# aask1357/fastenhancer

Measured on AMD Instinct MI355X. Metric: audio frames/sec (hop=256, 16kHz) FastEnhancer_B, higher is better.
Workload: dtype f32

## Files before the change

### fastenhancer_amd/_lib.py

```python
from __future__ import annotations

import ctypes
import os
from ctypes import POINTER, byref, c_char_p, c_double, c_float, c_int, c_longlong, c_size_t, c_void_p

HERE = os.path.dirname(os.path.abspath(__file__))
LIB_PATH = os.environ.get("FASTENHANCER_HIP_LIB") or os.path.join(HERE, "libfastenhancer_hip.so")
FE_MAX_KERNELS = 8

FE_OK = 0
FE_ARCH_FASTENHANCER = 0
FE_ARCH_BSRNN = 1
FE_ARCH_FSPEN = 2
FE_ARCH_LISENNET = 3
FE_OFFLINE_AUTO, FE_OFFLINE_FRAME_WALK, FE_OFFLINE_TIME_BATCHED = 0, 1, 2
FE_STEP_KERNEL_WAVES4, FE_STEP_KERNEL_WG8, FE_STEP_KERNEL_WG8_PERSIST = 0, 1, 2
FE_ACT_SILU, FE_ACT_RELU, FE_ACT_LEAKY_RELU, FE_ACT_ELU, FE_ACT_GELU, FE_ACT_GELU_TANH = 0, 1, 2, 3, 4, 5
FE_MASK_NONE, FE_MASK_SIGMOID, FE_MASK_TANH = 0, 1, 2
FE_AUDIO_F32, FE_AUDIO_S16 = 0, 1


class fe_config(ctypes.Structure):
    _fields_ = [
        ("arch", c_int), ("n_fft", c_int), ("hop_size", c_int), ("win_size", c_int),
# ... 64 lines not shown
    "fe_offline": (c_int, [c_void_p, c_void_p, c_int, c_int, c_void_p, c_void_p, c_void_p, c_void_p]),
    "fe_offline_ragged_work_floats": (c_size_t, [c_void_p, c_int, c_int]),
    "fe_offline_ragged": (c_int, [c_void_p, c_void_p, c_size_t, POINTER(c_int), c_int, c_void_p, c_size_t, c_void_p, c_void_p, c_void_p]),
    "fe_stft_step": (c_int, [c_void_p, c_void_p, c_size_t, c_void_p, c_void_p, c_void_p, c_int, c_void_p]),
    "fe_istft_step": (c_int, [c_void_p, c_void_p, c_void_p, c_void_p, c_void_p, c_size_t, c_int, c_void_p]),
    "fe_stft_offline": (c_int, [c_void_p, c_void_p, c_int, c_int, c_int, c_int, c_void_p, c_void_p]),
    "fe_istft_offline": (c_int, [c_void_p, c_void_p, c_int, c_int, c_int, c_int, c_void_p, c_void_p, c_void_p]),
    "fe_flops_per_frame": (c_double, [c_void_p]),
    "fe_debug_stages": (c_int, [c_void_p]),
    "fe_debug_stage": (c_int, [c_void_p, c_int, POINTER(c_char_p), POINTER(c_int), POINTER(c_int), POINTER(c_size_t)]),
    "fe_debug_floats": (c_size_t, [c_void_p]),
    "fe_debug_step": (c_int, [c_void_p, c_void_p, c_size_t, c_void_p, c_void_p, c_size_t, c_int, c_void_p, c_void_p]),
    "fe_profile_step": (c_int, [c_void_p, c_void_p, c_size_t, c_void_p, c_void_p, c_size_t, c_int, c_int, c_void_p, c_void_p]),
    "fe_debug_poison_lds": (c_int, [c_void_p]),
    "fe_debug_pack_weights": (c_int, [c_void_p, c_void_p, c_size_t, c_void_p, c_size_t, POINTER(c_size_t)]),
    "fe_last_error": (c_char_p, []),
    "fe_version": (c_char_p, []),
    "fe_build_key": (c_char_p, []),
}

_lib = None


class FEError(RuntimeError):
    pass


def load() -> ctypes.CDLL:
    global _lib
    if _lib is not None:
# ... 24 lines not shown
```

### fastenhancer_amd/csrc/fe_api.hip

```cpp
#include <hip/hip_runtime.h>

#include <algorithm>
#include <cmath>
#include <cstdarg>
#include <cstdio>
#include <cstdlib>
#include <cstring>
#include <string>
#include <vector>

#include "../../include/fastenhancer_hip.h"
#include "fe_fragments.h"
#include "fe_impl.h"
#include "bsrnn_kernels.hip.h"
#include "fspen_kernels.hip.h"
#include "lisennet_kernels.hip.h"
#include "stft_kernels.hip.h"

namespace fe {
namespace {
struct KernelLog { const char* name[16]; int n; };
thread_local KernelLog g_klog{};
}
void note_kernel(const char* name) {
// ... 408 lines not shown
            for (int g = 0; g < 3; ++g) {
                pack_1x1(o.blk_wih[k] + g * gsz, wih + (size_t)g * C2 * C2, C2, C2);
                pack_1x1(o.blk_whh[k] + g * gsz, whh + (size_t)g * C2 * C2, C2, C2);
                p.raw(o.blk_bih[k] + g * bsz, C2, bih + g * C2);
                p.raw(o.blk_bhh[k] + g * bsz, C2, bhh + g * C2);
            }
        }
        if (o.u8_gx[k] != 0) {
            const float* wih = S(key("rnn.weight_ih_l0"));
            const float* whh = S(key("rnn.weight_hh_l0"));
            const float* bih = S(key("rnn.bias_ih_l0"));
            const float* bhh = S(key("rnn.bias_hh_l0"));
            const int NG = C2 / 16, R = C2 % 16, NT = 3 * NG + 1, KS = C2 / 4;
            auto pack_u8 = [&](int off, int ntiles, const float* w, auto&& wrow, auto&& bias, auto&& rscale) {
                p.tiles(off, ntiles, KS, [&](int t, int c, int kk) { const int row = wrow(t, c); return row >= 0 ? w[(size_t)row * C2 + kk] * rscale(row) : 0.0f; });
                p.rows((size_t)off + (size_t)ntiles * KS * 64, ntiles, [&](int t, int c) { const int row = wrow(t, c); return row >= 0 ? bias(t, c) * rscale(row) : 0.0f; });
            };
            auto one = [](int) { return 1.0f; };
            auto gscale = [&](int row) { return row < 2 * C2 ? fe::kGateRZ : fe::kGateN; };
            auto grow = [&](int t, int c) -> int {
                if (t < 3 * NG) return (t % 3) * C2 + 16 * (t / 3) + c;
                return c < 3 * R ? (c / R) * C2 + 16 * NG + c % R : -1;
            };
            auto shared = [&](int t) { return t < 3 * NG && t % 3 < 2; };
            pack_u8(o.u8_gx[k], NT, wih, grow, [&](int t, int c) { const int r = grow(t, c); return bih[r] + (shared(t) ? bhh[r] : 0.0f); }, gscale);
            pack_u8(o.u8_gh[k], NT, whh, grow, [&](int t, int c) { const int r = grow(t, c); return shared(t) ? 0.0f : bhh[r]; }, gscale);
            auto plain = [&](int ncols) { return [ncols](int t, int c) { return 16 * t + c < ncols ? 16 * t + c : -1; }; };
            const float* f1b = S(key("rnn_fc.bias"));
            const float* f2b = S(key("attn_fc.bias"));
            pack_u8(o.u8_f1[k], fe::ceil_div(C2, 16), S(key("rnn_fc.weight")), plain(C2), [&](int t, int c) { return f1b[16 * t + c]; }, one);
            pack_1x1(o.u8_q[k], S(key("attn.qkv.weight")), C2, 3 * C2);
// ... 486 lines not shown
    return rc;
}

int fe_debug_pack_weights(fe_handle* h, const float* blob_host, size_t nfloats, float* out_host, size_t capacity, size_t* packed_floats) {
    if (!h || !blob_host) return fail(FE_ERR_INVALID_ARG, "null argument");
    if (nfloats != h->blob_floats) return fail(FE_ERR_INVALID_ARG, "blob has %zu floats, expected %zu", nfloats, h->blob_floats);
    std::vector<float> packed;
    const int rc = pack_blob(h, blob_host, &packed);
    if (rc != FE_OK) return rc;
    if (out_host && capacity < packed.size()) return fail(FE_ERR_INVALID_ARG, "output holds %zu floats, the packed buffer has %zu", capacity, packed.size());
    if (packed_floats) *packed_floats = packed.size();
    if (out_host) std::memcpy(out_host, packed.data(), packed.size() * sizeof(float));
    return FE_OK;
}

static const char* banks_unsupported(const fe_handle* h) {
    switch (h->cfg.arch) {
    case FE_ARCH_BSRNN: return "BSRNN";
    case FE_ARCH_FSPEN: return "FSPEN";
    case FE_ARCH_LISENNET: return "LiSenNet";
    default: return h->d.BD ? "noncausal FastEnhancer" : nullptr;
    }
}

int fe_weight_banks(const fe_handle* h) { return h ? h->n_banks : 0; }

int fe_set_weight_banks(fe_handle* h, int n_banks, void* stream) {
    if (!h) return fail(FE_ERR_INVALID_ARG, "null handle");
    if (n_banks < 1 || n_banks > FE_MAX_WEIGHT_BANKS)
        return fail(FE_ERR_INVALID_ARG, "fe_set_weight_banks: n_banks %d outside [1, FE_MAX_WEIGHT_BANKS = %d]", n_banks, FE_MAX_WEIGHT_BANKS);
// ... 1311 lines not shown
```

### fastenhancer_amd/csrc/fe_fragments.h

```cpp
#pragma once

#include <cstddef>
#include <vector>

namespace fe {
namespace frag {

enum Order { kPlain, kK4 };

constexpr size_t plain_index(int tile, int KS, int ks, int lane) { return ((size_t)tile * KS + ks) * 64 + lane; }
constexpr size_t k4_index(int tile, int KS, int ks, int lane) { return (((size_t)tile * (KS / 4) + ks / 4) * 64 + lane) * 4 + ks % 4; }
constexpr int lane_r(int lane) { return lane % 16; }
constexpr int lane_k(int ks, int lane) { return 4 * ks + lane / 16; }

struct Buffer {
    std::vector<float> v;
    explicit Buffer(size_t floats = 0) : v(floats, 0.0f) {}
    float& operator[](size_t i) { return v[i]; }
    size_t size() const { return v.size(); }
    int alloc(size_t n) {
        const size_t off = (v.size() + 63) & ~(size_t)63;
        v.resize(off + n, 0.0f);
        return (int)off;
    }
// ... 12 lines not shown
                    v[off + (O == kK4 ? k4_index(t, KS, ks, lane) : plain_index(t, KS, ks, lane))] = f(t, lane_r(lane), lane_k(ks, lane));
    }
    template <Order O = kPlain, class F>
    void pack_a(size_t off, int Mrows, int K, F&& Amk) {
        tiles<O>(off, (Mrows + 15) / 16, K / 4, [&](int t, int r, int k) { return 16 * t + r < Mrows ? Amk(16 * t + r, k) : 0.0f; });
    }
    template <Order O = kPlain, class F>
    void pack_b(size_t off, int K, int Ncols, F&& Bkn) {
        tiles<O>(off, (Ncols + 15) / 16, K / 4, [&](int t, int r, int k) { return 16 * t + r < Ncols ? Bkn(k, 16 * t + r) : 0.0f; });
    }
    template <class F>
    void rows(size_t off, int NT, F&& f) {
        for (int t = 0; t < NT; ++t)
            for (int r = 0; r < 16; ++r) v[off + (size_t)t * 16 + r] = f(t, r);
    }
    template <class TileMap>
    void regroup_k4(size_t dst, size_t src, int ntiles, int KS, int k0, int nk, TileMap&& src_tile) {
        for (int t = 0; t < ntiles; ++t)
            for (int ks = 0; ks < nk; ++ks)
                for (int lane = 0; lane < 64; ++lane)
                    v[dst + (size_t)t * nk * 64 + (ks < nk / 4 * 4 ? k4_index(0, nk, ks, lane) : plain_index(0, nk, ks, lane))] =
                        v[src + plain_index(src_tile(t), KS, k0 + ks, lane)];
    }
    void regroup_k4(size_t dst, size_t src, int ntiles, int KS, int k0, int nk) { regroup_k4(dst, src, ntiles, KS, k0, nk, [](int t) { return t; }); }
};

}
}
```

### fastenhancer_amd/csrc/fe_frame8.hip.h

```cpp
#pragma once
#include "fe_kernels.hip.h"

namespace fe {

constexpr int kThreads8 = 512;
constexpr int kWaves8 = 8;

template <class S>
struct Wg8 {
    using L = Lds<S>;
    static constexpr bool MDFT = (S::NFFT == 512) || (S::C1 < 128);
    static constexpr bool OK0 = L::STAGED && L::SKIPS_LDS && S::GFLAT && S::KT == 1 && S::LOW == 0 && !S::FRNN && !S::TATT && !S::LN && !S::BIDIR &&
                               S::G8P && S::MTC == 4 && S::MT2 == 2 && MDFT && !L::PERHEAD && S::NFFT == kThreads8 && S::NTPW2 == 1;
    static constexpr int NTA = (S::NTC + 1) / 2, NTB = S::NTC - NTA;
    static constexpr int N2A = (S::NT2 + 1) / 2, N2B = S::NT2 - N2A;
    static constexpr int NPW = ceil_div(ceil_div(Pack<S>::umax(), 256), kWaves8);
    static constexpr int HPT = ceil_div(S::F2 * S::C2, kThreads8);
    static constexpr int SLOT = S::U8_SLOT;
    static constexpr int WB0 = L::NOSTAGE_TOTAL, WB1 = WB0 + 2 * SLOT;
    static constexpr int LDM = 13;
    static constexpr int MXB = L::NOSTAGE_TOTAL + 4 * SLOT, MX_FLOATS = round_up(4 * 16 * LDM + 8, 4), MXF = MXB + 4 * 16 * LDM;
    static constexpr int HST = MXB + MX_FLOATS;
    static constexpr bool HSTASH = (size_t)(HST + S::KB * S::F2 * S::C2) * 4 <= 160 * 1024;
    static constexpr size_t BYTES = (size_t)(HST + (HSTASH ? S::KB * S::F2 * S::C2 : 0)) * 4;
// ... 11 lines not shown
    return q;
}
__device__ __forceinline__ f32x4 lds_v4(const LdsF* p) { return *reinterpret_cast<const LdsV4*>(p); }
template <int NPW, int NP>
struct Stage8 : StageSide<NPW, NP, kWaves8> {
    LdsF* w;
    __device__ __forceinline__ void commit() const {
        using B = StageSide<NPW, NP, kWaves8>;
#pragma unroll
        for (int i = 0; i < B::NPI; ++i) {
            const int p = this->j->wave + kWaves8 * i;
            if (kWaves8 * i + kWaves8 - 1 < NP || p < NP) *reinterpret_cast<LdsV4*>(w + i * (kWaves8 * 256)) = this->j->r[i];
        }
    }
};
__device__ __forceinline__ f32x4 lds_splat(const float* p) {
    const float b = *p;
    return f32x4{b, b, b, b};
}

template <class S, int NT, int J0, int KS, int NCOLS, int LDO, bool ACT, class AF, class BF, class BI, class SIDE>
__device__ __forceinline__ void conv8(AF&& af, BF&& bf, BI&& bias, const SIDE& side, LdsF* dst, int lane, float ap = 0.0f) {
    if constexpr (NT > 0) {
        const int li = lane & 15;
        f32x4 acc[1][NT];
#pragma unroll
        for (int j = 0; j < NT; ++j) acc[0][j] = bias(J0 + j);
        mma_panel<1, NT, KS, Lds<S>::PDK>(acc, [&](int, int ks) { return af(ks); }, [&](int j, int ks) { return bf(J0 + j, ks); }, side);
        side.commit();
#pragma unroll
        for (int j = 0; j < NT; ++j) {
            const int col = 16 * (J0 + j) + li;
            if (col < NCOLS) {
#pragma unroll
// ... 3 lines not shown
                    dst[r * LDO + 16 * (J0 + j)] = v;
                }
            }
        }
    } else {
        constexpr int NSG = (KS + 3) / 4;
#pragma unroll
        for (int g = 0; g < NSG; ++g) side(g, NSG);
        side.commit();
    }
}
template <class S, int NA, int NB, int KS, int NCOLS, int LDO, bool ACT, class AF, class BF, class BI, class SIDE>
__device__ __forceinline__ void conv8_pair(int wh, AF&& af, BF&& bf, BI&& bias, const SIDE& side, LdsF* dst, int lane, float ap = 0.0f) {
    if (wh == 0) conv8<S, NA, 0, KS, NCOLS, LDO, ACT>(af, bf, bias, side, dst, lane, ap);
    else conv8<S, NB, NA, KS, NCOLS, LDO, ACT>(af, bf, bias, side, dst, lane, ap);
}

template <class S, bool DBG, bool PERSIST, bool SLOT = false, bool HIO = false, bool STRM = false, bool BANK = false>
__global__ void __launch_bounds__(kThreads8) __attribute__((amdgpu_waves_per_eu(2, 2))) fe_frame8_kernel(typename KernelArgs<SLOT, STRM>::type a_in) {
    static_assert(Wg8<S>::OK, "fe_frame8_kernel: shape outside the 512-thread kernel's plan");
    static_assert(!BANK || STRM, "weight banks: the packet-audio instantiations only");
    static_assert(!HIO || (SLOT && !DBG), "host audio: slotted production instantiations only");
    static_assert(!STRM || HIO, "packet audio: the host-audio instantiations only");
    typename KernelArgs<SLOT, STRM>::type a = a_in;
    if constexpr (STRM) a.T = 1;
#ifdef FE_PROBE_HOT
    if constexpr (!DBG) a.dbg = nullptr;
#else
    if constexpr (!DBG) { a.dbg = nullptr; a.clk = nullptr; }
#endif
// ... 43 lines not shown
    wb.k4d = 0;
    float ap = 0.0f;
    if constexpr (S::EPP) ap = wp[o.act_p];
    LdsF* const wl0 = lds_window(smem + W8::WB0 + lane);
    LdsF* const wl1 = lds_window(smem + W8::WB1 + lane);
    LdsF* const stG = lds_window(smem + L::HL + (16 * (wave0 & 1) + 4 * (lane >> 4)) * LDX + 16 * (wave0 >> 1) + (lane & 15));
    LdsF* const stS = lds_window(smem + W8::HST + (16 * (wave0 & 1) + 4 * (lane >> 4)) * C2 + 16 * (wave0 >> 1) + (lane & 15));
    LdsF* const sw0 = lds_window(smem + W8::WB0 + wave0 * 256 + lane * 4);
    LdsF* const sw1 = lds_window(smem + W8::WB1 + wave0 * 256 + lane * 4);
    auto swin = [&](int dst_floats) { return dst_floats >= W8::WB1 ? sw1 + (dst_floats - W8::WB1) : sw0 + (dst_floats - W8::WB0); };
    LdsF* const wq0 = lds_window(smem + W8::WB0 + 4 * (lane & 15));
    LdsF* const wq1 = lds_window(smem + W8::WB1 + 4 * (lane & 15));
    LdsF* const stC = lds_window(smem + (16 * (wave0 & 3) + 4 * (lane >> 4)) * LDC + (lane & 15));
    LdsF* const stX = lds_window(smem + L::X + (16 * (wave0 >> 2) + 4 * (lane >> 4)) * LDX +
                                 (16 * (wave0 & 3) + (lane & 15) < C2 ? 16 * (wave0 & 3) + (lane & 15) : C2));

    float* sc = smem + L::SC;
    float* Ebuf = smem + L::E;
    float* W0 = smem + L::W0;
    float* W1 = smem + L::W1;
    float2* tw = reinterpret_cast<float2*>(smem + L::TW);
    constexpr int NPW = W8::NPW;
    DmaJobT<NPW> job;
    job.l = smem + W8::WB0;
    job.rsrc = wb.rsrc;
    job.soff = (o.u_off[0] + wave * 256) * 4;
    job.wave = wave;
    job.lane = lane;
    typename Dft<S>::FwdConst dc;
    float fv = 0.0f, fw = 0.0f;
// ... 195 lines not shown
                const float* const t0 = in + (16 * ws + li) * LDC + lg;
                conv8_pair<S, W8::NTA, W8::NTB, 3 * S::KS_C, C1, LDC, true>(
                    wh, [&](int ks) { return t0[(ks / S::KS_C) * LDC + 4 * (ks % S::KS_C)]; },
                    [&](int j, int ks) -> float { return wl_[o.enc_w[l] - ub_ + (j * (3 * S::KS_C) + ks) * 64]; },
                    [&](int j) { return lds_v4(wq_ + (o.enc_b[l] - ub_ + j * 64)); }, stage, stC + (L::E + (l + 1) * S::ACT + LDC), lane, ap);
            }
            if (l == 0) FE_CLK(42);
            __syncthreads();
            if (l == 0) FE_CLK(43);
            dbg_dump<S, NTH>(a, b, 3 + l, out + LDC, LDC);
        });

        float* Xb = smem + L::X;
        float* Hl = smem + L::HL;
        float* Hs = smem + L::HS;
        float* Gi = smem + L::GI;
        float* Y1 = smem + L::Y1;
        float* Y2 = smem + L::Y2;

        FE_CLK(5);
        constexpr int NTPW3 = S::NTPW3;
        constexpr int HPT = W8::HPT;
        constexpr int K2 = S::KS_2;
        f32x4 xr;
        const int g_rt = wave & 1;
        const int g_t0 = wave < 4 ? 3 * (wave >> 1) : 3 * S::G8_NG;
        const float* const sGx = smem + W8::WB0 + 1 * W8::SLOT;
        const float* const sGh = smem + W8::WB0 + 3 * W8::SLOT;
        const float* const sF = smem + W8::WB0 + 0 * W8::SLOT;
        static_assert(W8::WB1 == W8::WB0 + 2 * W8::SLOT, "slots 2 (qkv) and 3 are reached through WB1's window");
        constexpr int NPWB = W8::NPWB;
        DmaJobT<NPWB> jb1, jb2;
        jb1.rsrc = wb.rsrc; jb1.wave = wave; jb1.lane = lane; jb1.l = smem; jb1.soff = 0;
        jb2 = jb1;
        auto stage_to = [&](DmaJobT<NPWB>& j, int src_floats, int dst_floats) { j.l = smem + dst_floats; j.soff = (src_floats + wave * 256) * 4; };
        constexpr int u8_stride = S::KB > 1 ? o.u8_gx[1] - o.u8_gx[0] : 0;
        using StG = Stage8<NPWB, S::U8_G / 256>;
        using StF = Stage8<NPWB, S::U8_F / 256>;
        using StQ = Stage8<NPWB, S::U8_Q / 256>;
        float pe_r[4];
        int hs_off[HPT];
#pragma unroll
        for (int q = 0; q < HPT; ++q) {
            const int i = tid + q * NTH, f = i / C2;
            hs_off[q] = i < F2 * C2 ? f * LDX + (i - f * C2) : C2;
// ... 53 lines not shown
            const int ub = k * u8_stride;
            if (k == 0) FE_CLK(20);
            {
                stage_to(jb1, o.u8_f1[0] + ub, W8::WB0 + 0 * W8::SLOT);
                stage_to(jb2, o.u8_q[0] + ub, W8::WB0 + 2 * W8::SLOT);
                const StF st1{{&jb1}, swin(W8::WB0 + 0 * W8::SLOT)};
                const StQ st2{{&jb2}, swin(W8::WB0 + 2 * W8::SLOT)};
                const auto sideg = side2(st1, st2);
                if (k == 0) {
#pragma unroll
                    for (int r = 0; r < 4; ++r) {
                        const int row = 16 * wh + 4 * lg + r, col = 16 * ws + li;
                        pe_r[r] = wb.gather_g(o.blk_pe + (row < F2 ? row : F2 - 1) * C2 + (col < C2 ? col : C2 - 1));
                    }
                }
                const float* xa = Xb + (16 * g_rt + li) * LDX + lg;
                const float* ha = Hs + (16 * g_rt + li) * LDX + lg;
                const LdsF* const wx = wl0 + (1 * W8::SLOT + g_t0 * (K2 * 64));
                const LdsF* const wh_ = wl1 + (1 * W8::SLOT + g_t0 * (K2 * 64));
                const float* bx = sGx + S::G8_NT * K2 * 64 + g_t0 * 16 + li;
                const float* bh = sGh + S::G8_NT * K2 * 64 + g_t0 * 16 + li;
                __builtin_amdgcn_sched_barrier(0);
                if (k == 0) FE_CLK(45);
                if (wave < 4) {
                    const int ch = 16 * (wave >> 1) + li;
                    float hprev[4];
#pragma unroll
                    for (int r = 0; r < 4; ++r) hprev[r] = stG[(L::HS - L::HL) + r * LDX];
                    f32x4 ar = lds_splat(bx), az = lds_splat(bx + 16);
                    f32x4 anx = lds_splat(bx + 32), anh = lds_splat(bh + 32);
                    mma_panel_sel<1, 3, 2 * K2, PDK>(
                        [&](int, int j, int ks) -> f32x4& { return j == 0 ? ar : (j == 1 ? az : (ks < K2 ? anx : anh)); },
                        [&](int, int ks) { return ks < K2 ? xa[4 * ks] : ha[4 * (ks - K2)]; },
                        [&](int j, int ks) -> float { return ks < K2 ? wx[(j * K2 + ks) * 64] : wh_[(j * K2 + (ks - K2)) * 64]; }, sideg);
                    __builtin_amdgcn_sched_barrier(0);
                    if (k == 0) FE_CLK(46);
                    float hn[4];
#pragma unroll
                    for (int r = 0; r < 4; ++r) {
                        const float rr = sigmoid_pre(ar[r]);
                        const float zz = sigmoid_pre(az[r]);
                        const float nn = tanh_pre(__builtin_fmaf(rr, anh[r], anx[r]));
                        hn[r] = __builtin_fmaf(zz, hprev[r] - nn, nn);
                    }
                    if (16 * g_rt + 4 * lg < F2) {
// ... 2 lines not shown
                            const int row = 16 * g_rt + 4 * lg + r;
                            stG[r * LDX] = hn[r];
                            if constexpr (W8::HSTASH) stS[k * (F2 * C2) + r * C2] = hn[r];
                            else hg[row * C2 + ch] = hn[r];
                        }
                    }
                } else {
                    constexpr int R = S::G8_R, LDM = W8::LDM;
                    const bool hhalf = wave >= 6;
                    float* mx = smem + W8::MXB + ((hhalf ? 2 : 0) + g_rt) * (16 * LDM);
                    int* mflag = reinterpret_cast<int*>(smem + W8::MXF) + g_rt;
                    const int seq = fc * S::KB + k + 1;
                    f32x4 s0, s1 = f32x4{0.0f, 0.0f, 0.0f, 0.0f};
                    __builtin_amdgcn_s_setprio(3);
                    if (!hhalf) {
                        s0 = lds_splat(bx);
                        mma_panel_sel<1, 1, K2, PDK>([&](int, int, int ks) -> f32x4& { return (ks & 1) ? s1 : s0; },
                                                     [&](int, int ks) { return xa[4 * ks]; }, [&](int, int ks) -> float { return wx[ks * 64]; }, sideg);
                    } else {
                        s0 = lds_splat(bh);
                        mma_panel_sel<1, 1, K2, PDK>([&](int, int, int ks) -> f32x4& { return ((ks + K2) & 1) ? s1 : s0; },
                                                     [&](int, int ks) { return ha[4 * ks]; }, [&](int, int ks) -> float { return wh_[ks * 64]; }, sideg);
                    }
                    s0 += s1;
                    __builtin_amdgcn_sched_barrier(0);
                    if (k == 0) FE_CLK(46);
                    if (li < 3 * R) {
#pragma unroll
                        for (int r = 0; r < 4; ++r) mx[(4 * lg + r) * LDM + li] = s0[r];
                    }
                    if (!hhalf) {
                        __atomic_signal_fence(__ATOMIC_SEQ_CST);
                        __builtin_amdgcn_s_waitcnt(0xc07f);
                        if (lane == 0) __hip_atomic_store(mflag, seq, __ATOMIC_RELAXED, __HIP_MEMORY_SCOPE_WORKGROUP);
                        __atomic_signal_fence(__ATOMIC_SEQ_CST);
// ... 17 lines not shown
                        if (live) {
                            Hl[(16 * g_rt + row) * LDX + ch] = hn;
                            if constexpr (W8::HSTASH) smem[W8::HST + k * (F2 * C2) + (16 * g_rt + row) * C2 + ch] = hn;
                            else hg[(16 * g_rt + row) * C2 + ch] = hn;
                        }
                    }
                    __builtin_amdgcn_s_setprio(0);
                }
                st1.commit();
                st2.commit();
            }
            if (k == 0) FE_CLK(47);
            __syncthreads();
            if (k == 0) FE_CLK(21);
            if (k == 0) FE_CLK(22);
            const int ntf = ws < S::NT2 ? ws : S::NT2 - 1;
            {
                stage_to(jb1, o.u8_gx[0] + ub + u8_stride, W8::WB0 + 1 * W8::SLOT);
                const StG stn{{&jb1}, swin(W8::WB0 + 1 * W8::SLOT)};
                f32x4 acc[1][1];
                acc[0][0] = lds_splat(sF + S::NT2 * K2 * 64 + ntf * 16 + li);
                const float* hla = Hl + (16 * wh + li) * LDX + lg;
                const LdsF* const wf = wl0 + ntf * (K2 * 64);
                if (k + 1 < S::KB) {
                    mma_panel<1, 1, K2, PDK>(acc, [&](int, int ks) { return hla[4 * ks]; }, [&](int, int ks) -> float { return wf[ks * 64]; }, stn);
                    stn.commit();
                } else
                    mma_panel<1, 1, K2, PDK>(acc, [&](int, int ks) { return hla[4 * ks]; }, [&](int, int ks) -> float { return wf[ks * 64]; }, NoSide{});
#pragma unroll
                for (int r = 0; r < 4; ++r) {
                    float v = acc[0][0][r] + xr[r];
                    if (k == 0) v += pe_r[r];
                    xr[r] = v;
                    stX[r * LDX] = v;
                }
            }
            __syncthreads();
            dbg_dump<S, NTH>(a, b, 4 + S::NL + 2 * k, Xb, LDX);
            if (k == 0) FE_CLK(23);
            {
                stage_to(jb1, o.u8_f2[0] + ub, W8::WB0 + 0 * W8::SLOT);
                const StF st1{{&jb1}, swin(W8::WB0 + 0 * W8::SLOT)};
                f32x4 acc[1][NTPW3];
                acc_init_zero<1, NTPW3>(acc);
                __builtin_amdgcn_sched_barrier(0);
                if (k == 0) FE_CLK(50);
                const float* xa = Xb + (16 * wh + li) * LDX + lg;
                mma_panel<1, NTPW3, K2, PDK>(acc, [&](int, int ks) { return xa[4 * ks]; },
                                             [&](int j, int ks) -> float {
                                                 int nt = ws + 4 * j;
                                                 nt = nt < S::NT3 ? nt : S::NT3 - 1;
                                                 return wl1[(nt * K2 + ks) * 64];
                                             }, st1);
                st1.commit();
                __builtin_amdgcn_sched_barrier(0);
                if (k == 0) FE_CLK(51);
                float* gdst = Gi + (16 * wh + 4 * lg) * LDG + 16 * ws + li;
#pragma unroll
                for (int j = 0; j < NTPW3; ++j)
                    if (ws + 4 * j < S::NT3) {
#pragma unroll
                        for (int r = 0; r < 4; ++r) gdst[r * LDG + 64 * j] = acc[0][j][r];
                    }
                __builtin_amdgcn_sched_barrier(0);
                if (k == 0) FE_CLK(52);
            }
            __syncthreads();
            if (k == 0) FE_CLK(24);
            attention_head<S, 1, LDG>(Gi, Hl, ws * 3 * HD, ws, wh, 1, lane);
            __syncthreads();
            if (k == 0) FE_CLK(25);
            {
                float hpre[HPT];
                if (k + 1 < S::KB) {
                    const float* hgn = hg + (size_t)nst * (F2 * C2);
#pragma unroll
                    for (int q = 0; q < HPT; ++q) { const int i = tid + q * NTH; hpre[q] = hgn[i < F2 * C2 ? i : F2 * C2 - 1]; }
                }
                f32x4 acc[1][1];
                acc[0][0] = lds_splat(sF + S::NT2 * K2 * 64 + ntf * 16 + li);
                const float* hla = Hl + (16 * wh + li) * LDX + lg;
                const LdsF* const wf = wl0 + ntf * (K2 * 64);
                if (k + 1 < S::KB) {
                    stage_to(jb1, o.u8_gh[0] + ub + u8_stride, W8::WB0 + 3 * W8::SLOT);
                    const StG stn{{&jb1}, swin(W8::WB0 + 3 * W8::SLOT)};
                    mma_panel<1, 1, K2, PDK>(acc, [&](int, int ks) { return hla[4 * ks]; }, [&](int, int ks) -> float { return wf[ks * 64]; }, stn);
                    stn.commit();
                } else {
                    stage_to(jb1, o.u_off[S::U_RFPOST], W8::WB1);
                    const Stage8<NPWB, o.u_size[S::U_RFPOST] / 256> stn{{&jb1}, swin(W8::WB1)};
                    mma_panel<1, 1, K2, PDK>(acc, [&](int, int ks) { return hla[4 * ks]; }, [&](int, int ks) -> float { return wf[ks * 64]; }, stn);
                    stn.commit();
                }
                if (k + 1 < S::KB) {
#pragma unroll
                    for (int q = 0; q < HPT; ++q) Hs[hs_off[q]] = hpre[q];
                }
// ... 125 lines not shown
                    for (int f = tid; f < F0; f += NTH) {
                        float yr, yi;
                        limited_bin<S>(PT, sc, f, b0, b1, ctl.m_min, e, yr, yi);
                        q3[f] = yr;
                        q3[N / 2 + f] = yi;
                    }
                }
            }
        }
        __syncthreads();

        FE_CLK(11);
        {
            const float ow = wp[o.window_istft + tid];
            const float oc = tid < OVL ? cis[tid] : 0.0f;
            if (wave < 4) Dft<S>::template inverse<WSrc<true>, false>(q3, q0, q1, tw, idc, wb, o, wave, lane);
            __syncthreads();
            FE_CLK(12);
            const int pi = Dft<S>::pidx(tid & (Dft<S>::N1 - 1), tid / Dft<S>::N1);
            const float xo = (q0[pi] + q1[pi]) * ow + oc;
            if constexpr (STRM) {
                if (a.levels != nullptr) {
                    if (64 * wave < H) {
                        const float x = tid < H ? xo : 0.0f;
                        ctl.lv.out_ss = wave_sum(0.0f, x * x);
                        ctl.lv.out_pk = wave_max(0.0f, fabsf(x));
                    }
                    levels_put(PT, ctl.lv, wave, lane);
                }
                if (a.format) {
                    const int qv = pcm16_out(xo);
                    const int pw = pcm16_pair(qv, __shfl_down(qv, 1));
                    const int p1 = __shfl_down(pw, 2), p2 = __shfl_down(pw, 4), p3 = __shfl_down(pw, 6);
                    short* orow = reinterpret_cast<short*>(a.wav_out) + sv.out_off;
                    if (tid < H) {
// ... 58 lines not shown
```

### fastenhancer_amd/csrc/fe_kernels.hip.h

```cpp
#pragma once
#include <hip/hip_runtime.h>

#include <type_traits>
#include <utility>

#include "fe_launch.h"
#include "fe_handover.h"

#ifndef FE_OCC_SMALL
#define FE_OCC_SMALL 3
#endif
namespace fe {

typedef float f32x4 __attribute__((ext_vector_type(4)));

#define FE_MFMA(a, b, c) __builtin_amdgcn_mfma_f32_16x16x4f32((a), (b), (c), 0, 0, 0)

constexpr int FE_MODE_STREAM = 0, FE_MODE_SPEC = 1, FE_MODE_OFFLINE = 2;
constexpr int kThreads = 256;
constexpr int kWaves = 4;


template <class F, int... I>
__device__ __forceinline__ void static_for_impl(F& f, std::integer_sequence<int, I...>) { (f(std::integral_constant<int, I>{}), ...); }
// ... 45 lines not shown
    static constexpr int KS_C = C1 / 4;
    static constexpr int KS_2 = C2 / 4;
    static constexpr int NU = 6 + NL * (2 * KT + 1) + (LN ? 1 : 0);
    static constexpr int U_ENC = 1;
    static constexpr int U_RFPRE = 1 + NL * KT;
    static constexpr int U_RFPOST = 3 + NL * KT;
    static constexpr int U_DEC = 4 + NL * KT + (LN ? 1 : 0);
    static constexpr int U_POST = 4 + NL * (2 * KT + 1) + (LN ? 1 : 0);
    static constexpr int TKQ = (KT - 1) * (F0 / 4) * C1;
    static constexpr int NTPW2 = ceil_div(NT2, kWaves), NTPW3 = ceil_div(NT3, kWaves);
    static constexpr bool GFLAT = (C2 % 16 != 0) && (3 * NTPW3 + 2 * NTPW2) * KS_2 <= 160;
    static constexpr bool REGW = GFLAT || (NTPW2 * 6 + NTPW3 + 2 * NTPW2) * KS_2 <= 160;
    static constexpr int G8_NG = C2 / 16, G8_R = C2 % 16;
    static constexpr bool G8P = GFLAT && MT2 == 2 && G8_NG == 2 && G8_R > 0 && 3 * G8_R <= 16 && KT_ == 1 && FR_ == 0 && TA_ == 0 && LN_ == 0 && BD_ == 0;
    static constexpr int G8_NT = 3 * G8_NG + 1;
    static constexpr int U8_G = round_up(G8_NT * (C2 / 4) * 64 + G8_NT * 16, 256);
    static constexpr int U8_F = round_up(ceil_div(C2, 16) * (C2 / 4) * 64 + ceil_div(C2, 16) * 16, 256);
    static constexpr int U8_Q = round_up(ceil_div(3 * C2, 16) * (C2 / 4) * 64, 256);
    static constexpr int U8_SLOT = U8_G > U8_Q ? U8_G : U8_Q;
    static_assert(C1 % 4 == 0 && C2 % 4 == 0 && F2 % 4 == 0, "channel counts must be multiples of 4");
    static_assert(C2 % NH == 0, "C2 must be divisible by the 4 heads");
    static_assert(F1 % 64 == 0, "F1 must be a multiple of 64");
    static_assert(LOG2N > 0, "n_fft must be 512 or 1024");
};

struct PackedOffsets {
    int enc_pre_w, enc_pre_b;
    int enc_w[16], enc_b[8];
    int rfpre_lin, rfpre_w, rfpre_b;
    int blk_pe;
    int blk_stride;
    int blk_wih[8], blk_bih[8], blk_whh[8], blk_bhh[8];
// ... 893 lines not shown
            }
        float* P = jt ? P1 : P0;
#pragma unroll
        for (int i = 0; i < MT; ++i) {
            f32x4 e0 = {0.0f, 0.0f, 0.0f, 0.0f}, e1 = e0;
#pragma unroll
            for (int r = 0; r < 4; ++r) {
                e0 = FE_MFMA(hq[i][0][r], c.c4[r], e0);
                e1 = FE_MFMA(hq[i][1][r], c.c4[4 + r], e1);
            }
#pragma unroll
            for (int r = 0; r < 4; ++r) P[pidx(16 * i + 4 * lg + r, 16 * p + li)] = e0[r] + e1[r];
        }
        if constexpr (BAR) __syncthreads();
    }
};

template <class S, int NT, int KS_TOT, class WS>
struct ConvB {
    const WS& w;
    int w_off;
    mutable f32x4 cur[NT];
    static constexpr bool K4 = !std::is_same_v<std::remove_cv_t<WS>, WSrc<true>> && KS_TOT >= 4;
    __device__ __forceinline__ float operator()(int j, int ks) const {
        constexpr int CK4 = Pack<S>::v.conv_k4_delta;
        if constexpr (K4 && CK4 != 0) {
            const int base = w_off + CK4 + j * (KS_TOT * 64);
            if (ks >= 4 * (KS_TOT / 4)) return w.at_g(base + ks * 64);
            if ((ks & 3) == 0) cur[j] = w.at_gv4(base + (ks >> 2) * 256, w.lane4 * 4);
            return cur[j][ks & 3];
// ... 2052 lines not shown
```

### include/fastenhancer_hip.h

```cpp
#ifndef FASTENHANCER_HIP_H
#define FASTENHANCER_HIP_H

#include <stddef.h>

#ifdef __cplusplus
extern "C" {
#endif

#define FE_OK 0
#define FE_ERR_INVALID_ARG (-1)
#define FE_ERR_UNSUPPORTED_CONFIG (-2)
#define FE_ERR_HIP (-3)
#define FE_ERR_NO_WEIGHTS (-4)

#define FE_ARCH_FASTENHANCER 0
#define FE_ARCH_BSRNN 1
#define FE_ARCH_FSPEN 2

#define FE_ARCH_LISENNET 3

#define FE_MAX_KERNELS 8

#define FE_ACT_SILU 0
#define FE_ACT_RELU 1
// ... 147 lines not shown
double fe_flops_per_frame(const fe_handle* h);

int fe_debug_stages(const fe_handle* h);
int fe_debug_stage(const fe_handle* h, int idx, const char** name, int* rows, int* cols, size_t* offset_floats);
size_t fe_debug_floats(const fe_handle* h);
int fe_debug_step(fe_handle* h, const float* wav_in_dev, size_t in_stride, float* state_dev,
                  float* wav_out_dev, size_t out_stride, int B, float* dbg_dev, void* stream);

int fe_profile_step(fe_handle* h, const float* wav_in_dev, size_t in_stride, float* state_dev,
                    float* wav_out_dev, size_t out_stride, int B, int T, unsigned long long* clk_dev, void* stream);

int fe_debug_poison_lds(void* stream);

int fe_debug_pack_weights(fe_handle* h, const float* blob_host, size_t nfloats, float* out_host, size_t capacity, size_t* packed_floats);

const char* fe_last_error(void);
const char* fe_version(void);
const char* fe_build_key(void);

#ifdef __cplusplus
}
#endif
#endif
```

Baseline: 8.423 million.

## Precompute LDS windows, vectorize bias splats, specialize attention and inverse-DFT gather

Moves the per-wave LDS address arithmetic for the GRU, FFN, QKV, attention and inverse-DFT stages into one set of windows computed at kernel entry. Biases are now packed four times per row so each can be read as one vector LDS load instead of a scalar splat. A dedicated single-tile attention routine and an inverse-DFT tail fed from a register gather replace the generic paths. A debug API reporting block-unit offsets is added. The aim is fewer address computations and scalar LDS reads in the per-hop kernel, at the cost of larger packed bias storage and more live registers.

```diff
diff --git a/fastenhancer_amd/_lib.py b/fastenhancer_amd/_lib.py
--- a/fastenhancer_amd/_lib.py
+++ b/fastenhancer_amd/_lib.py
@@ -102,6 +102,7 @@
     "fe_profile_step": (c_int, [c_void_p, c_void_p, c_size_t, c_void_p, c_void_p, c_size_t, c_int, c_int, c_void_p, c_void_p]),
     "fe_debug_poison_lds": (c_int, [c_void_p]),
     "fe_debug_pack_weights": (c_int, [c_void_p, c_void_p, c_size_t, c_void_p, c_size_t, POINTER(c_size_t)]),
+    "fe_debug_block_unit": (c_int, [c_void_p, c_int, c_int, POINTER(c_size_t), POINTER(c_int), POINTER(c_int)]),
     "fe_last_error": (c_char_p, []),
     "fe_version": (c_char_p, []),
     "fe_build_key": (c_char_p, []),
diff --git a/fastenhancer_amd/csrc/fe_api.hip b/fastenhancer_amd/csrc/fe_api.hip
--- a/fastenhancer_amd/csrc/fe_api.hip
+++ b/fastenhancer_amd/csrc/fe_api.hip
@@ -446,7 +446,7 @@
             const int NG = C2 / 16, R = C2 % 16, NT = 3 * NG + 1, KS = C2 / 4;
             auto pack_u8 = [&](int off, int ntiles, const float* w, auto&& wrow, auto&& bias, auto&& rscale) {
                 p.tiles(off, ntiles, KS, [&](int t, int c, int kk) { const int row = wrow(t, c); return row >= 0 ? w[(size_t)row * C2 + kk] * rscale(row) : 0.0f; });
-                p.rows((size_t)off + (size_t)ntiles * KS * 64, ntiles, [&](int t, int c) { const int row = wrow(t, c); return row >= 0 ? bias(t, c) * rscale(row) : 0.0f; });
+                p.rows4((size_t)off + (size_t)ntiles * KS * 64, ntiles, [&](int t, int c) { const int row = wrow(t, c); return row >= 0 ? bias(t, c) * rscale(row) : 0.0f; });
             };
             auto one = [](int) { return 1.0f; };
             auto gscale = [&](int row) { return row < 2 * C2 ? fe::kGateRZ : fe::kGateN; };
@@ -963,6 +963,21 @@
     return FE_OK;
 }
 
+int fe_debug_block_unit(const fe_handle* h, int block, int unit, size_t* offset_floats, int* tiles, int* ksteps) {
+    if (!h) return fail(FE_ERR_INVALID_ARG, "null handle");
+    if (!h->impl || !h->impl->off || h->impl->off->u8_gx[0] == 0)
+        return fail(FE_ERR_UNSUPPORTED_CONFIG, "fe_debug_block_unit: this model has no staged block units (the 512-thread per-hop kernel does not run it)");
+    if (block < 0 || block >= h->d.KB || unit < 0 || unit > 4) return fail(FE_ERR_INVALID_ARG, "fe_debug_block_unit: block %d, unit %d", block, unit);
+    const fe::PackedOffsets& o = *h->impl->off;
+    const int C2 = h->d.C2;
+    const int* const at[5] = {o.u8_gx, o.u8_gh, o.u8_f1, o.u8_q, o.u8_f2};
+    const int nt[5] = {3 * (C2 / 16) + 1, 3 * (C2 / 16) + 1, fe::ceil_div(C2, 16), fe::ceil_div(3 * C2, 16), fe::ceil_div(C2, 16)};
+    if (offset_floats) *offset_floats = (size_t)at[unit][block];
+    if (tiles) *tiles = nt[unit];
+    if (ksteps) *ksteps = C2 / 4;
+    return FE_OK;
+}
+
 static const char* banks_unsupported(const fe_handle* h) {
     switch (h->cfg.arch) {
     case FE_ARCH_BSRNN: return "BSRNN";
diff --git a/fastenhancer_amd/csrc/fe_fragments.h b/fastenhancer_amd/csrc/fe_fragments.h
--- a/fastenhancer_amd/csrc/fe_fragments.h
+++ b/fastenhancer_amd/csrc/fe_fragments.h
@@ -50,6 +50,14 @@
         for (int t = 0; t < NT; ++t)
             for (int r = 0; r < 16; ++r) v[off + (size_t)t * 16 + r] = f(t, r);
     }
+    template <class F>
+    void rows4(size_t off, int NT, F&& f) {
+        for (int t = 0; t < NT; ++t)
+            for (int c = 0; c < 16; ++c) {
+                const float b = f(t, c);
+                for (int r = 0; r < 4; ++r) v[off + ((size_t)t * 16 + c) * 4 + r] = b;
+            }
+    }
     template <class TileMap>
     void regroup_k4(size_t dst, size_t src, int ntiles, int KS, int k0, int nk, TileMap&& src_tile) {
         for (int t = 0; t < ntiles; ++t)
diff --git a/fastenhancer_amd/csrc/fe_frame8.hip.h b/fastenhancer_amd/csrc/fe_frame8.hip.h
--- a/fastenhancer_amd/csrc/fe_frame8.hip.h
+++ b/fastenhancer_amd/csrc/fe_frame8.hip.h
@@ -49,10 +49,6 @@
         }
     }
 };
-__device__ __forceinline__ f32x4 lds_splat(const float* p) {
-    const float b = *p;
-    return f32x4{b, b, b, b};
-}
 
 template <class S, int NT, int J0, int KS, int NCOLS, int LDO, bool ACT, class AF, class BF, class BI, class SIDE>
 __device__ __forceinline__ void conv8(AF&& af, BF&& bf, BI&& bias, const SIDE& side, LdsF* dst, int lane, float ap = 0.0f) {
@@ -86,6 +82,65 @@
 __device__ __forceinline__ void conv8_pair(int wh, AF&& af, BF&& bf, BI&& bias, const SIDE& side, LdsF* dst, int lane, float ap = 0.0f) {
     if (wh == 0) conv8<S, NA, 0, KS, NCOLS, LDO, ACT>(af, bf, bias, side, dst, lane, ap);
     else conv8<S, NB, NA, KS, NCOLS, LDO, ACT>(af, bf, bias, side, dst, lane, ap);
+}
+
+template <class S, int LDG, int PDK>
+__device__ __forceinline__ void attention8(const LdsF* kW, const LdsF* qW, const LdsF* (&vW)[S::MT2], LdsF* oW, int qt, int lane) {
+    constexpr int HD = S::HD, F2 = S::F2, LDX = S::LDX;
+    constexpr int KSD = ceil_div(HD, 4);
+    static_assert(HD <= 16 && F2 % 4 == 0, "attention8: one d tile, keys in groups of four");
+    const int li = lane & 15, lg = lane >> 4;
+    f32x4 sacc[S::MT2][1];
+    acc_init_zero<S::MT2, 1>(sacc);
+    mma_panel<S::MT2, 1, KSD, PDK>(
+        sacc, [&](int i, int ks) { return kW[(16 * i) * LDG + 4 * ks]; },
+        [&](int, int ks) {
+            const float v = qW[4 * ks];
+            return 4 * ks + lg < HD ? v : 0.0f;
+        }, NoSide{});
+    float av[S::MT2][4];
+#pragma unroll
+    for (int i = 0; i < S::MT2; ++i)
+#pragma unroll
+        for (int r = 0; r < 4; ++r) av[i][r] = vW[i][r * LDG];
+    const float scale = rsqrtf((float)HD) * 1.4426950408889634f;
+    float mx = -INFINITY;
+#pragma unroll
+    for (int i = 0; i < S::MT2; ++i) {
+        const bool padk = 16 * i + 4 * lg >= F2;
+#pragma unroll
+        for (int r = 0; r < 4; ++r) {
+            float sv = sacc[i][0][r];
+            if (16 * i + 15 >= F2) sv = padk ? -INFINITY : sv;
+            sacc[i][0][r] = sv;
+            mx = fmaxf(mx, sv);
+        }
+    }
+    mx = rows_allreduce(mx, [](float p, float q) { return fmaxf(p, q); }) * scale;
+    float sum = 0.0f;
+#pragma unroll
+    for (int i = 0; i < S::MT2; ++i)
+#pragma unroll
+        for (int r = 0; r < 4; ++r) {
+            float p = __builtin_amdgcn_exp2f(__builtin_fmaf(sacc[i][0][r], scale, -mx));
+            sacc[i][0][r] = p;
+            sum += p;
+        }
+    sum = rows_allreduce(sum, [](float p, float q) { return p + q; });
+    const float inv_sum = __builtin_amdgcn_rcpf(sum);
+    f32x4 oacc = {0.0f, 0.0f, 0.0f, 0.0f};
+#pragma unroll
+    for (int i = 0; i < S::MT2; ++i)
+#pragma unroll
+        for (int r = 0; r < 4; ++r) oacc = FE_MFMA(av[i][r], sacc[i][0][r], oacc);
+    const int q = 16 * qt + li;
+#pragma unroll
+    for (int r = 0; r < 4; ++r) {
+        const int d = 4 * lg + r;
+        float ov = oacc[r] * inv_sum;
+        asm volatile("" : "+v"(ov));
+        if (d < HD && q < F2) oW[r] = ov;
+    }
 }
 
 template <class S, bool DBG, bool PERSIST, bool SLOT = false, bool HIO = false, bool STRM = false, bool BANK = false>
@@ -159,6 +214,30 @@
     LdsF* const stC = lds_window(smem + (16 * (wave0 & 3) + 4 * (lane >> 4)) * LDC + (lane & 15));
     LdsF* const stX = lds_window(smem + L::X + (16 * (wave0 >> 2) + 4 * (lane >> 4)) * LDX +
                                  (16 * (wave0 & 3) + (lane & 15) < C2 ? 16 * (wave0 & 3) + (lane & 15) : C2));
+    constexpr int K2W = S::KS_2;
+    const int g_t0w = wave0 < 4 ? 3 * (wave0 >> 1) : 3 * S::G8_NG;
+    const int ntfw = (wave0 & 3) < S::NT2 ? (wave0 & 3) : S::NT2 - 1;
+    LdsF* const wG = lds_window(smem + W8::WB0 + 1 * W8::SLOT + g_t0w * (K2W * 64) + lane);
+    LdsF* const qG = lds_window(smem + W8::WB0 + 1 * W8::SLOT + S::G8_NT * K2W * 64 + g_t0w * 64 + 4 * (lane & 15));
+    LdsF* const wF = lds_window(smem + W8::WB0 + ntfw * (K2W * 64) + lane);
+    LdsF* const qF = lds_window(smem + W8::WB0 + S::NT2 * K2W * 64 + ntfw * 64 + 4 * (lane & 15));
+    LdsF* const wQ = lds_window(smem + W8::WB0 + 2 * W8::SLOT + (wave0 & 3) * (K2W * 64) + lane);
+    LdsF* const aG = lds_window(smem + L::X + (16 * (wave0 & 1) + (lane & 15)) * LDX + (lane >> 4));
+    LdsF* const aT = lds_window(smem + L::X + (16 * (wave0 >> 2) + (lane & 15)) * LDX + (lane >> 4));
+    LdsF* const stQ = lds_window(smem + L::GI + (16 * (wave0 >> 2) + 4 * (lane >> 4)) * LDG + 16 * (wave0 & 3) + (lane & 15));
+    constexpr int HOFF = 3 * HD;
+    LdsF* const atK = lds_window(smem + L::GI + (lane & 15) * LDG + (wave0 & 3) * HOFF + HD + (lane >> 4));
+    LdsF* const atQ = lds_window(smem + L::GI + (16 * (wave0 >> 2) + (lane & 15)) * LDG + (wave0 & 3) * HOFF + (lane >> 4));
+    const LdsF* atV[S::MT2];
+#pragma unroll
+    for (int i = 0; i < S::MT2; ++i) {
+        const int key = 16 * i + 4 * (lane >> 4);
+        atV[i] = lds_window(smem + L::GI + (key < F2 - 4 ? key : F2 - 4) * LDG + (wave0 & 3) * HOFF + 2 * HD + ((lane & 15) < HD ? (lane & 15) : HD - 1));
+    }
+    LdsF* const dfA = lds_window(smem + L::FFT_B + N + (32 * (lane >> 4) + 16 * (wave0 & 1) + (lane & 15)));
+    LdsF* const dfB = lds_window(smem + L::FFT_B + N + N / 2 - (32 * (lane >> 4) + 16 * (wave0 & 1) + (lane & 15)));
+    LdsF* const dfP = lds_window(smem + L::FFT_A + Dft<S>::pidx(tid0 & (Dft<S>::N1 - 1), tid0 / Dft<S>::N1));
+    LdsF* const atO = lds_window(smem + L::HL + (16 * (wave0 >> 2) + (lane & 15)) * LDX + (wave0 & 3) * HD + 4 * (lane >> 4));
 
     float* sc = smem + L::SC;
     float* Ebuf = smem + L::E;
@@ -384,7 +463,6 @@
         float* Xb = smem + L::X;
         float* Hl = smem + L::HL;
         float* Hs = smem + L::HS;
-        float* Gi = smem + L::GI;
         float* Y1 = smem + L::Y1;
         float* Y2 = smem + L::Y2;
 
@@ -394,11 +472,8 @@
         constexpr int K2 = S::KS_2;
         f32x4 xr;
         const int g_rt = wave & 1;
-        const int g_t0 = wave < 4 ? 3 * (wave >> 1) : 3 * S::G8_NG;
-        const float* const sGx = smem + W8::WB0 + 1 * W8::SLOT;
-        const float* const sGh = smem + W8::WB0 + 3 * W8::SLOT;
-        const float* const sF = smem + W8::WB0 + 0 * W8::SLOT;
-        static_assert(W8::WB1 == W8::WB0 + 2 * W8::SLOT, "slots 2 (qkv) and 3 are reached through WB1's window");
+        static_assert(W8::WB1 == W8::WB0 + 2 * W8::SLOT, "slots 2 (qkv) and 3 lie 2 SLOT behind slots 0 and 1");
+        static_assert(K2 == K2W, "the block windows' tile stride");
         constexpr int NPWB = W8::NPWB;
         DmaJobT<NPWB> jb1, jb2;
         jb1.rsrc = wb.rsrc; jb1.wave = wave; jb1.lane = lane; jb1.l = smem; jb1.soff = 0;
@@ -482,12 +557,12 @@
                         pe_r[r] = wb.gather_g(o.blk_pe + (row < F2 ? row : F2 - 1) * C2 + (col < C2 ? col : C2 - 1));
                     }
                 }
-                const float* xa = Xb + (16 * g_rt + li) * LDX + lg;
-                const float* ha = Hs + (16 * g_rt + li) * LDX + lg;
-                const LdsF* const wx = wl0 + (1 * W8::SLOT + g_t0 * (K2 * 64));
-                const LdsF* const wh_ = wl1 + (1 * W8::SLOT + g_t0 * (K2 * 64));
-                const float* bx = sGx + S::G8_NT * K2 * 64 + g_t0 * 16 + li;
-                const float* bh = sGh + S::G8_NT * K2 * 64 + g_t0 * 16 + li;
+                const LdsF* const xa = aG;
+                const LdsF* const ha = aG + (L::HS - L::X);
+                const LdsF* const wx = wG;
+                const LdsF* const wh_ = wG + 2 * W8::SLOT;
+                const LdsF* const bx = qG;
+                const LdsF* const bh = qG + 2 * W8::SLOT;
                 __builtin_amdgcn_sched_barrier(0);
                 if (k == 0) FE_CLK(45);
                 if (wave < 4) {
@@ -495,8 +570,8 @@
                     float hprev[4];
 #pragma unroll
                     for (int r = 0; r < 4; ++r) hprev[r] = stG[(L::HS - L::HL) + r * LDX];
-                    f32x4 ar = lds_splat(bx), az = lds_splat(bx + 16);
-                    f32x4 anx = lds_splat(bx + 32), anh = lds_splat(bh + 32);
+                    f32x4 ar = lds_v4(bx), az = lds_v4(bx + 64);
+                    f32x4 anx = lds_v4(bx + 128), anh = lds_v4(bh + 128);
                     mma_panel_sel<1, 3, 2 * K2, PDK>(
                         [&](int, int j, int ks) -> f32x4& { return j == 0 ? ar : (j == 1 ? az : (ks < K2 ? anx : anh)); },
                         [&](int, int ks) { return ks < K2 ? xa[4 * ks] : ha[4 * (ks - K2)]; },
@@ -529,11 +604,11 @@
                     f32x4 s0, s1 = f32x4{0.0f, 0.0f, 0.0f, 0.0f};
                     __builtin_amdgcn_s_setprio(3);
                     if (!hhalf) {
-                        s0 = lds_splat(bx);
+                        s0 = lds_v4(bx);
                         mma_panel_sel<1, 1, K2, PDK>([&](int, int, int ks) -> f32x4& { return (ks & 1) ? s1 : s0; },
                                                      [&](int, int ks) { return xa[4 * ks]; }, [&](int, int ks) -> float { return wx[ks * 64]; }, sideg);
                     } else {
-                        s0 = lds_splat(bh);
+                        s0 = lds_v4(bh);
                         mma_panel_sel<1, 1, K2, PDK>([&](int, int, int ks) -> f32x4& { return ((ks + K2) & 1) ? s1 : s0; },
                                                      [&](int, int ks) { return ha[4 * ks]; }, [&](int, int ks) -> float { return wh_[ks * 64]; }, sideg);
                     }
@@ -581,14 +656,13 @@
             __syncthreads();
             if (k == 0) FE_CLK(21);
             if (k == 0) FE_CLK(22);
-            const int ntf = ws < S::NT2 ? ws : S::NT2 - 1;
             {
                 stage_to(jb1, o.u8_gx[0] + ub + u8_stride, W8::WB0 + 1 * W8::SLOT);
                 const StG stn{{&jb1}, swin(W8::WB0 + 1 * W8::SLOT)};
                 f32x4 acc[1][1];
-                acc[0][0] = lds_splat(sF + S::NT2 * K2 * 64 + ntf * 16 + li);
-                const float* hla = Hl + (16 * wh + li) * LDX + lg;
-                const LdsF* const wf = wl0 + ntf * (K2 * 64);
+                acc[0][0] = lds_v4(qF);
+                const LdsF* const hla = aT + (L::HL - L::X);
+                const LdsF* const wf = wF;
                 if (k + 1 < S::KB) {
                     mma_panel<1, 1, K2, PDK>(acc, [&](int, int ks) { return hla[4 * ks]; }, [&](int, int ks) -> float { return wf[ks * 64]; }, stn);
                     stn.commit();
@@ -612,29 +686,24 @@
                 acc_init_zero<1, NTPW3>(acc);
                 __builtin_amdgcn_sched_barrier(0);
                 if (k == 0) FE_CLK(50);
-                const float* xa = Xb + (16 * wh + li) * LDX + lg;
-                mma_panel<1, NTPW3, K2, PDK>(acc, [&](int, int ks) { return xa[4 * ks]; },
-                                             [&](int j, int ks) -> float {
-                                                 int nt = ws + 4 * j;
-                                                 nt = nt < S::NT3 ? nt : S::NT3 - 1;
-                                                 return wl1[(nt * K2 + ks) * 64];
-                                             }, st1);
+                static_assert(4 * NTPW3 * K2 * 64 <= W8::SLOT, "qkv: the tiles past NT3 stay inside the staging slot");
+                mma_panel<1, NTPW3, K2, PDK>(acc, [&](int, int ks) { return aT[4 * ks]; },
+                                             [&](int j, int ks) -> float { return wQ[((4 * j) * K2 + ks) * 64]; }, st1);
                 st1.commit();
                 __builtin_amdgcn_sched_barrier(0);
                 if (k == 0) FE_CLK(51);
-                float* gdst = Gi + (16 * wh + 4 * lg) * LDG + 16 * ws + li;
 #pragma unroll
                 for (int j = 0; j < NTPW3; ++j)
                     if (ws + 4 * j < S::NT3) {
 #pragma unroll
-                        for (int r = 0; r < 4; ++r) gdst[r * LDG + 64 * j] = acc[0][j][r];
+                        for (int r = 0; r < 4; ++r) stQ[r * LDG + 64 * j] = acc[0][j][r];
                     }
                 __builtin_amdgcn_sched_barrier(0);
                 if (k == 0) FE_CLK(52);
             }
             __syncthreads();
             if (k == 0) FE_CLK(24);
-            attention_head<S, 1, LDG>(Gi, Hl, ws * 3 * HD, ws, wh, 1, lane);
+            attention8<S, LDG, L::PDK>(atK, atQ, atV, atO, wh, lane);
             __syncthreads();
             if (k == 0) FE_CLK(25);
             {
@@ -645,9 +714,9 @@
                     for (int q = 0; q < HPT; ++q) { const int i = tid + q * NTH; hpre[q] = hgn[i < F2 * C2 ? i : F2 * C2 - 1]; }
                 }
                 f32x4 acc[1][1];
-                acc[0][0] = lds_splat(sF + S::NT2 * K2 * 64 + ntf * 16 + li);
-                const float* hla = Hl + (16 * wh + li) * LDX + lg;
-                const LdsF* const wf = wl0 + ntf * (K2 * 64);
+                acc[0][0] = lds_v4(qF);
+                const LdsF* const hla = aT + (L::HL - L::X);
+                const LdsF* const wf = wF;
                 if (k + 1 < S::KB) {
                     stage_to(jb1, o.u8_gh[0] + ub + u8_stride, W8::WB0 + 3 * W8::SLOT);
                     const StG stn{{&jb1}, swin(W8::WB0 + 3 * W8::SLOT)};
@@ -803,11 +872,30 @@
         {
             const float ow = wp[o.window_istft + tid];
             const float oc = tid < OVL ? cis[tid] : 0.0f;
-            if (wave < 4) Dft<S>::template inverse<WSrc<true>, false>(q3, q0, q1, tw, idc, wb, o, wave, lane);
+            if (wave < 4) {
+                static_assert(Dft<S>::N1 == 16 && Dft<S>::KC == 8, "the gather below: N = 512");
+                static_assert((size_t)(L::FFT_B + 2 * N) * 4 < W8::BYTES, "the zeroed lane's read of Y[N] stays inside the workgroup's LDS");
+                const bool z0 = (lane == 0) && !(wave & 1);
+                float yq[8];
+#pragma unroll
+                for (int ks = 0; ks < 8; ++ks) {
+                    const int hb = ks >> 2, c = ks & 3;
+                    float v;
+                    if (c < 2) {
+                        v = dfA[hb * (N / 2) + 128 * c];
+                        if (hb == 1 && c == 0) v = z0 ? 0.0f : v;
+                    } else {
+                        v = dfB[hb * (N / 2) - 128 * (c - 2)];
+                        if (hb == 1) v = -v;
+                        if (c == 2) v = z0 ? 0.0f : v;
+                    }
+                    yq[ks] = v;
+                }
+                Dft<S>::template inverse_tail<WSrc<true>, false>(yq, q0, q1, tw, idc, wb, o, wave, lane);
+            }
             __syncthreads();
             FE_CLK(12);
-            const int pi = Dft<S>::pidx(tid & (Dft<S>::N1 - 1), tid / Dft<S>::N1);
-            const float xo = (q0[pi] + q1[pi]) * ow + oc;
+            const float xo = (dfP[0] + dfP[N]) * ow + oc;
             if constexpr (STRM) {
                 if (a.levels != nullptr) {
                     if (64 * wave < H) {
diff --git a/fastenhancer_amd/csrc/fe_kernels.hip.h b/fastenhancer_amd/csrc/fe_kernels.hip.h
--- a/fastenhancer_amd/csrc/fe_kernels.hip.h
+++ b/fastenhancer_amd/csrc/fe_kernels.hip.h
@@ -83,8 +83,8 @@
     static constexpr int G8_NG = C2 / 16, G8_R = C2 % 16;
     static constexpr bool G8P = GFLAT && MT2 == 2 && G8_NG == 2 && G8_R > 0 && 3 * G8_R <= 16 && KT_ == 1 && FR_ == 0 && TA_ == 0 && LN_ == 0 && BD_ == 0;
     static constexpr int G8_NT = 3 * G8_NG + 1;
-    static constexpr int U8_G = round_up(G8_NT * (C2 / 4) * 64 + G8_NT * 16, 256);
-    static constexpr int U8_F = round_up(ceil_div(C2, 16) * (C2 / 4) * 64 + ceil_div(C2, 16) * 16, 256);
+    static constexpr int U8_G = round_up(G8_NT * (C2 / 4) * 64 + G8_NT * 64, 256);
+    static constexpr int U8_F = round_up(ceil_div(C2, 16) * (C2 / 4) * 64 + ceil_div(C2, 16) * 64, 256);
     static constexpr int U8_Q = round_up(ceil_div(3 * C2, 16) * (C2 / 4) * 64, 256);
     static constexpr int U8_SLOT = U8_G > U8_Q ? U8_G : U8_Q;
     static_assert(C1 % 4 == 0 && C2 % 4 == 0 && F2 % 4 == 0, "channel counts must be multiples of 4");
@@ -1008,6 +1008,46 @@
         }
         if constexpr (BAR) __syncthreads();
     }
+    template <class WS, bool BAR = true, class OFF = PackedOffsets>
+    __device__ static __forceinline__ void inverse_tail(const float (&yq)[KC], float* P0, float* P1, const float2* tw, const InvConst& c,
+                                                        const WS& wb, const OFF& o, int wave, int lane) {
+        const int li = lane & 15, lg = lane >> 4, p = wave >> 1, jt = wave & 1;
+        f32x4 h[1][2 * MT];
+        acc_init_zero<1, 2 * MT>(h);
+        mma_panel<1, 2 * MT, KC, PDK>(h, [&](int, int ks) { return yq[ks]; },
+                                 [&](int j, int ks) {
+                                     if constexpr (PRELOAD3) return c.c3[j][ks];
+                                     else return wb.at_g(o.dft3 + (j * KC + ks) * 64);
+                                 }, NoSide{});
+        float hq[MT][2][4];
+        float2 tq[MT][4];
+#pragma unroll
+        for (int i = 0; i < MT; ++i)
+#pragma unroll
+            for (int r = 0; r < 4; ++r) tq[i][r] = twid(tw, (16 * i + li) * (16 * jt + 4 * lg + r));
+#pragma unroll
+        for (int i = 0; i < MT; ++i)
+#pragma unroll
+            for (int r = 0; r < 4; ++r) {
+                const float2 t = tq[i][r];
+                const float hr = h[0][i][r], hi = h[0][MT + i][r];
+                hq[i][0][r] = hr * t.x + hi * t.y;
+                hq[i][1][r] = hi * t.x - hr * t.y;
+            }
+        float* P = jt ? P1 : P0;
+#pragma unroll
+        for (int i = 0; i < MT; ++i) {
+            f32x4 e0 = {0.0f, 0.0f, 0.0f, 0.0f}, e1 = e0;
+#pragma unroll
+            for (int r = 0; r < 4; ++r) {
+                e0 = FE_MFMA(hq[i][0][r], c.c4[r], e0);
+                e1 = FE_MFMA(hq[i][1][r], c.c4[4 + r], e1);
+            }
+#pragma unroll
+            for (int r = 0; r < 4; ++r) P[pidx(16 * i + 4 * lg + r, 16 * p + li)] = e0[r] + e1[r];
+        }
+        if constexpr (BAR) __syncthreads();
+    }
 };
 
 template <class S, int NT, int KS_TOT, class WS>
diff --git a/include/fastenhancer_hip.h b/include/fastenhancer_hip.h
--- a/include/fastenhancer_hip.h
+++ b/include/fastenhancer_hip.h
@@ -185,6 +185,8 @@
 
 int fe_debug_pack_weights(fe_handle* h, const float* blob_host, size_t nfloats, float* out_host, size_t capacity, size_t* packed_floats);
 
+int fe_debug_block_unit(const fe_handle* h, int block, int unit, size_t* offset_floats, int* tiles, int* ksteps);
+
 const char* fe_last_error(void);
 const char* fe_version(void);
 const char* fe_build_key(void);
```

New measurement: 8.486 million (median of 6 runs). No clear change (+0.7%).
